# magicat777/Audio-Analyzer-OMEGA

Hardware: AMD Instinct MI355X
Metric: audio frames/sec (multi-res FFT + LUFS + TruePeak) at 1/2/4/8 MI355X (higher is better)
Workload: dtype f32; 1 GPU; cfg2: 256 stereo frames x 16384 samples per GPU; MRFFT 16k/8k/4k/1k + combine(512) + K-weighted LUFS + 4x true peak + meter aggregates; channel_frames_per_gpu=512, frame_samples=16384, target_bins=512, parallelism=frames sharded over 1 GPU(s)

## Files before the change

### audio-analyzer-omega_amd/csrc/capi.cpp

```cpp
#include <hip/hip_runtime.h>

#include <algorithm>
#include <cmath>
#include <cstdarg>
#include <cstdio>
#include <cstdlib>
#include <cstring>
#include <exception>
#include <map>
#include <new>
#include <string>
#include <vector>

#include "../../include/omega.h"
#include "params.hpp"

namespace omega {
hipError_t launch_spectral(int W, const SpectralParams& p, hipStream_t s);
hipError_t launch_mrfft(const SpectralParams& p, hipStream_t s);
hipError_t launch_mrfft_range(const SpectralParams& p, int r0, int r1, hipStream_t s);
hipError_t launch_mrfft_independent(const SpectralParams& p, hipStream_t s);
hipError_t launch_truepeak(int W, const SpectralParams& p, hipStream_t s);
hipError_t launch_truepeak_rf(int W, const SpectralParams& p, hipStream_t s, int extra_lds = 0);
hipError_t launch_mrfft_rf(int n, const SpectralParams& p, int r, hipStream_t s);
// ... 942 lines not shown
    p.seg_post_target = c->seg_par[b];
    v.push_back(p);
    c->cur = b;
  }
  return v;
}

int meters_enqueue(omega_ctx* c, const float* lufs, const float* tp, int64_t n_frames, double* out,
                   hipStream_t stream, hipEvent_t tp_ready, unsigned* wait_ctr = nullptr, unsigned wait_target = 0) {
  bool first = true;
  for (MeterPrepParams p : meter_chunks(c, lufs, tp, n_frames, out)) {
    if (first && wait_ctr) {
      p.wait_ctr = wait_ctr;
      p.wait_target = wait_target;
    }
    HIPC(c, launch_meter_prep(p, stream));
    if (tp_ready && first) HIPC(c, hipStreamWaitEvent(stream, tp_ready, 0));
    HIPC(c, launch_meter_query(p, stream));
    first = false;
  }
  return 0;
}

int flush_meters(omega_ctx* c) {
  if (!c->pend) return 0;
  HIPC(c, hipSetDevice(c->device));
  BatchPlan bp{};
  bp.q_begin = 0;
  bp.q_n = c->pend_nq;
  bp.seg_start[0] = bp.seg_start[1] = bp.multi_start = c->pend_nq;
  SpectralParams sp{};
  KWeightParams kp{};
  const hipError_t le = launch_batch(sp, kp, bp, c->pend_mq, c->pend_nq, c->stream);
  if (le != hipSuccess) return fail(c, OMEGA_EHIP, "meter segment launch: %s", hipGetErrorString(le));
  c->pend = false;
  c->seg_par[c->pend_par] = c->seg_issued + (unsigned)c->pend_nq;
  c->seg_issued += (unsigned)c->pend_nq;
  return 0;
}

bool batch_eligible(omega_ctx* c, const SpectralParams& sp, const KWeightParams& kp, int W, bool do_res, hipStream_t s,
                    int* mr) {
  *mr = -1;
  if (W != 16384 || (c->cap && s == c->cap)) return false;
  if ((kp.lufs_out || kp.weighted_out) && kp.mode != 0) return false;
  if (!do_res) return true;
  if (!c->res_independent) return false;
  for (int r = 0; r < sp.n_res; ++r) {
    if (!sp.comb_out && !sp.res[r].mag_out) continue;
    const int n = sp.res[r].n;
    if (n == 16384) {
      if (*mr >= 0 || !((sp.rf_sizes >> 14) & 1)) return false;
      *mr = r;
    } else if (n < 512 || n > 8192) {
      return false;
    }
  }
  return true;
}

int enqueue_batch(omega_ctx* c, SpectralParams sp, KWeightParams kp, int W, int64_t n_frames, const float* lufs,
                  const float* tp, double* meters, hipStream_t s, int mr, bool do_tp, bool do_kw, bool fold) {
  (void)W;
  const int64_t n = sp.n_cf;
  BatchPlan bp{};
  int seg[2][3], ns[2] = {0, 0};
  auto add = [&](int sg, int role, bool on) {
    if (on) seg[sg][ns[sg]++] = role;
  };
  add(0, 0, do_kw);
  add(0, 2, mr >= 0);
  add(1, 1, do_tp);
  const int64_t groups = (n + 7) / 8;
  int64_t end = 0;
  for (int sg = 0; sg < 2; ++sg) {
    bp.n_roles[sg] = ns[sg] ? ns[sg] : 1;
    for (int i = 0; i < 3; ++i) bp.roles[sg][i] = i < ns[sg] ? seg[sg][i] : 0;
    end += ns[sg] ? 8 * ns[sg] * groups : 0;
    if (end > 0x7FFFFFFF) return fail(c, OMEGA_EINVAL, "batch of %lld channel-frames too large", (long long)n);
    bp.seg_begin[sg + 1] = (int)end;
  }
  bp.mr_res = mr < 0 ? 0 : mr;
  int64_t nwg = 0;
  for (int r = 0; r < sp.n_res; ++r) {
    if (r == mr || (!sp.comb_out && !sp.res[r].mag_out)) continue;
    const int K = sp.res[r].n / 2;
    const int G = K / 16 < 64 ? 64 : K / 16;
    const int fpw = 512 / G;
    bp.multi.res[bp.multi.n_seg] = r;
    bp.multi.wg_begin[bp.multi.n_seg] = (int)nwg;
    ++bp.multi.n_seg;
    nwg += (n + fpw - 1) / fpw;
  }
  const bool in_grid = meters && do_tp && do_kw && n_frames > 0 && n_frames <= kChunkFrames;
  const int64_t n_mq = in_grid ? std::min<int64_t>((n + kBatchWaves - 1) / kBatchWaves, kMeterWgs) : 0;
  fold = fold && in_grid;
  const int64_t q_n = fold ? (c->pend ? c->pend_nq : 0) : n_mq;
  bp.pat = 1;
  bp.multi_n = (int)nwg;
  bp.seg_start[0] = 0;
  bp.seg_start[1] = bp.seg_begin[1];
  bp.multi_start = bp.seg_begin[2];
  const int64_t body_end = end + nwg;
  bp.q_begin = (int)body_end;
  bp.q_n = (int)q_n;
  if (fold) bp.q_begin = bp.multi_start;
  const int64_t grid = body_end + q_n;
  if (grid > 0x7FFFFFFF) return fail(c, OMEGA_EINVAL, "batch of %lld channel-frames too large", (long long)n);
  MeterPrepParams mq{};
  std::vector<MeterPrepParams> mc;
  if (in_grid) {
    const int a = c->cur;
    const unsigned seg_par_was = c->seg_par[a ^ 1];
    if (fold && c->pend) c->seg_par[c->pend_par] = c->seg_issued + (unsigned)c->pend_nq;
    const int cur_was = c->cur;
    mc = meter_chunks(c, lufs, tp, n_frames, meters);
    MeterPrepParams p = mc[0];
    p.q_done = c->d_kw_done + 3;
    const size_t mir_n = (size_t)kChunkFrames * c->cfg.n_channels;
    if (fold && !c->d_mirror) {
      HIPC(c, hipMalloc(&c->d_mirror, 2 * mir_n * sizeof(unsigned long long)));
      HIPC(c, hipMemset(c->d_mirror, 0, 2 * mir_n * sizeof(unsigned long long)));
    }
    const bool mirror = fold;
    const unsigned gen_was = c->mirror_gen;
    if (mirror) {
      c->mirror_gen = c->mirror_gen == 0xFFFFFFFFu ? 2u : c->mirror_gen + 1;
      kp.lufs_mirror = c->d_mirror + (c->mirror_gen & 1) * mir_n;
      kp.mirror_gen = c->mirror_gen;
      p.lufs_mirror = kp.lufs_mirror;
      p.mirror_gen = c->mirror_gen;
    } else {
      kp.kw_done = c->d_kw_done;
      c->kw_issued += (unsigned)n;
      p.wait_ctr = c->d_kw_done;
      p.wait_target = c->kw_issued;
    }
    if (fold && c->tail_ok == 0) {
      int ok = 0;
      HIPC(c, hipDeviceGetAttribute(&ok, hipDeviceAttributeCanUseStreamWaitValue, c->device));
      c->tail_ok = -1;
      if (ok && hipExtMallocWithFlags(reinterpret_cast<void**>(&c->d_tail), 8, hipMallocSignalMemory) == hipSuccess) {
        HIPC(c, hipMemset(c->d_tail, 0, 8));
        c->tail_issued = 0;
        c->tail_ok = 1;
      }
    }
    const bool tail = fold && c->tail_ok > 0;
    if (tail) bp.tail_ctr = c->d_tail;
    if (!fold) HIPC(c, launch_meter_prep(p, c->fork[0]));
    c->side_meters = true;
    mq = mc[0];
    mq.start_ctr = c->d_kw_done + 3;
    mq.start_target = c->prep_issued + (unsigned)p.C;
    if (!fold) {
      sp.tp_done = c->d_kw_done + 2;
      mq.join_ctr = c->d_kw_done + 2;
      mq.join_target = c->tp_issued + (unsigned)n;
    }
    const hipError_t le = launch_batch(sp, kp, bp, fold ? c->pend_mq : mq, (int)grid, s);
    if (le != hipSuccess) {
      if (!fold) {
        (void)hipMemcpy(c->d_kw_done, &c->kw_issued, sizeof(unsigned), hipMemcpyHostToDevice);
        c->prep_issued += (unsigned)p.C;
      } else {
        c->mirror_gen = gen_was;
        c->seg_par[a ^ 1] = seg_par_was;
        c->cur = cur_was;
// ... 2104 lines not shown
```

### audio-analyzer-omega_amd/csrc/fft.hpp

```cpp
#pragma once
#include <hip/hip_runtime.h>
#include <type_traits>
#include <utility>

namespace omega {

constexpr int NT = 256;

template <int A, int B, class F>
__device__ __forceinline__ void static_for(F&& f) {
  if constexpr (A < B) {
    f(std::integral_constant<int, A>{});
    static_for<A + 1, B>(f);
  }
}

constexpr int ilog2(int v) { return v <= 1 ? 0 : 1 + ilog2(v >> 1); }

template <int R>
constexpr int brev(int m) {
  int r = 0;
  for (int b = 0; b < ilog2(R); ++b) r |= ((m >> b) & 1) << (ilog2(R) - 1 - b);
  return r;
}
// ... 70 lines not shown
  for (int n1 = 0; n1 < 4; ++n1) {
    const float2 a0 = v[n1], a1 = v[n1 + 4], a2 = v[n1 + 8], a3 = v[n1 + 12];
    const float2 s02 = make_float2(a0.x + a2.x, a0.y + a2.y), d02 = make_float2(a0.x - a2.x, a0.y - a2.y);
    const float2 s13 = make_float2(a1.x + a3.x, a1.y + a3.y), d13 = make_float2(a1.x - a3.x, a1.y - a3.y);
    v[n1 + 0] = make_float2(s02.x + s13.x, s02.y + s13.y);
    v[n1 + 8] = make_float2(s02.x - s13.x, s02.y - s13.y);
    v[n1 + 4] = make_float2(d02.x + d13.y, d02.y - d13.x);
    v[n1 + 12] = make_float2(d02.x - d13.y, d02.y + d13.x);
  }
  float2 y[16];
#pragma unroll
  for (int i = 0; i < 16; ++i) y[4 * (i & 3) + (i >> 2)] = v[i];
  {
    const float2 a0 = y[0], a1 = y[4], a2 = y[8], a3 = y[12];
    const float2 s02 = make_float2(a0.x + a2.x, a0.y + a2.y), d02 = make_float2(a0.x - a2.x, a0.y - a2.y);
    const float2 s13 = make_float2(a1.x + a3.x, a1.y + a3.y), d13 = make_float2(a1.x - a3.x, a1.y - a3.y);
    v[0] = make_float2(s02.x + s13.x, s02.y + s13.y);
    v[8] = make_float2(s02.x - s13.x, s02.y - s13.y);
    v[4] = make_float2(d02.x + d13.y, d02.y - d13.x);
    v[12] = make_float2(d02.x - d13.y, d02.y + d13.x);
  }
  {
    const float2 a0 = y[1], a1 = y[5], a2 = y[9], a3 = y[13];
    const float p2x = a2.x + a2.y, p2y = a2.y - a2.x, p3x = a3.x + a3.y, p3y = a3.y - a3.x;
    const float2 s02 = make_float2(fmaf(h, p2x, a0.x), fmaf(h, p2y, a0.y));
    const float2 d02 = make_float2(fmaf(-h, p2x, a0.x), fmaf(-h, p2y, a0.y));
    const float2 e = make_float2(fmaf(h, p3x, a1.x), fmaf(h, p3y, a1.y));
    const float2 f = make_float2(fmaf(-h, p3x, a1.x), fmaf(-h, p3y, a1.y));
    const float ux = fmaf(t8, e.y, e.x), uy = fmaf(-t8, e.x, e.y);
    const float wx = fmaf(t8, f.y, f.x), wy = fmaf(-t8, f.x, f.y);
    v[1] = make_float2(fmaf(c8, ux, s02.x), fmaf(c8, uy, s02.y));
    v[9] = make_float2(fmaf(-c8, ux, s02.x), fmaf(-c8, uy, s02.y));
    v[5] = make_float2(fmaf(c8, wy, d02.x), fmaf(-c8, wx, d02.y));
    v[13] = make_float2(fmaf(-c8, wy, d02.x), fmaf(c8, wx, d02.y));
  }
  {
    const float2 a0 = y[2], a1 = y[6], a2 = y[10], a3 = y[14];
    const float2 s02 = make_float2(a0.x + a2.y, a0.y - a2.x), d02 = make_float2(a0.x - a2.y, a0.y + a2.x);
    const float2 e = make_float2(a1.x + a3.y, a1.y - a3.x), f = make_float2(a1.x - a3.y, a1.y + a3.x);
    const float pex = e.x + e.y, pey = e.y - e.x, pfx = f.x + f.y, pfy = f.y - f.x;
    v[2] = make_float2(fmaf(h, pex, s02.x), fmaf(h, pey, s02.y));
    v[10] = make_float2(fmaf(-h, pex, s02.x), fmaf(-h, pey, s02.y));
    v[6] = make_float2(fmaf(h, pfy, d02.x), fmaf(-h, pfx, d02.y));
    v[14] = make_float2(fmaf(-h, pfy, d02.x), fmaf(h, pfx, d02.y));
  }
  {
    const float2 a0 = y[3], a1 = y[7], a2 = y[11], a3 = y[15];
    const float q2s = a2.x + a2.y, q2d = a2.y - a2.x, q3s = a3.x + a3.y, q3d = a3.y - a3.x;
    const float2 s02 = make_float2(fmaf(h, q2d, a0.x), fmaf(-h, q2s, a0.y));
    const float2 d02 = make_float2(fmaf(-h, q2d, a0.x), fmaf(h, q2s, a0.y));
    const float2 e = make_float2(fmaf(h, q3d, a1.x), fmaf(-h, q3s, a1.y));
    const float2 f = make_float2(fmaf(-h, q3d, a1.x), fmaf(h, q3s, a1.y));
    const float ux = fmaf(t8, e.x, e.y), uy = fmaf(t8, e.y, -e.x);
    const float wx = fmaf(t8, f.x, f.y), wy = fmaf(t8, f.y, -f.x);
    v[3] = make_float2(fmaf(c8, ux, s02.x), fmaf(c8, uy, s02.y));
    v[11] = make_float2(fmaf(-c8, ux, s02.x), fmaf(-c8, uy, s02.y));
    v[7] = make_float2(fmaf(c8, wy, d02.x), fmaf(-c8, wx, d02.y));
    v[15] = make_float2(fmaf(-c8, wy, d02.x), fmaf(c8, wx, d02.y));
  }
}

template <int R>
__device__ __forceinline__ void dft_nat(float2* v) {
  if constexpr (R == 16) {
    dft16_fma(v);
  } else {
    dft_dif<R>(v);
    float2 o[R];
    static_for<0, R>([&](auto m) { o[m] = v[brev<R>(m)]; });
    static_for<0, R>([&](auto m) { v[m] = o[m]; });
  }
}

template <int NS, int R>
__device__ __forceinline__ int swz(int i) {
  if constexpr (NS >= 16 || NS == 0) {
    return i;
  } else {
    constexpr int a = ilog2(NS * R), c = ilog2(NS), m = 16 / NS - 1;
    return i ^ (((i >> a) & m) << c);
  }
}

template <int NP>
struct TwReg {
  float2 w[NP > 0 ? NP : 1];
  __device__ __forceinline__ void launder() {
    static_for<0, (NP > 0 ? NP : 1)>([&](auto i) { asm volatile("" : "+v"(w[i].x), "+v"(w[i].y)); });
  }
};

template <int K, int R, int NS, int NTH, bool SYNC_MID, class Load, class Store>
__device__ __forceinline__ void fft_pass(float2 w1, int tid, Load&& load, Store&& store) {
  constexpr int NB = K / R;
  constexpr int B = (NB + NTH - 1) / NTH;
  static_assert(NS == 1 || B == 1, "twiddled passes: one butterfly per thread");
  float2 v[B][R];
  static_for<0, B>([&](auto b) {
    const int j = tid + b * NTH;
    if (NB % NTH == 0 || j < NB) static_for<0, R>([&](auto r) { v[b][r] = load(j + r * NB); });
  });
  if constexpr (SYNC_MID) __syncthreads();
  static_for<0, B>([&](auto b) {
    const int j = tid + b * NTH;
    if (NB % NTH == 0 || j < NB) {
      const int k = j & (NS - 1);
      if constexpr (NS > 1) {
        float2 w = w1;
        static_for<1, R>([&](auto r) {
          v[b][r] = cmul(v[b][r], w);
          if constexpr (r + 1 < R) w = cmul(w, w1);
        });
      }
      dft_nat<R>(v[b]);
      const int base = (j / NS) * NS * R + k;
      static_for<0, R>([&](auto m) { store(base + m * NS, v[b][m]); });
    }
  });
}

template <int K, int NTH, int I, int NS, int PNS, int PR, int... Rs>
struct StockhamChain;
template <int K, int NTH, int I, int NS, int PNS, int PR>
struct StockhamChain<K, NTH, I, NS, PNS, PR> {
  template <class TW>
  static __device__ __forceinline__ void load_tw(const float2*, int, TW&) {}
  template <bool FIRST, bool LAST, bool PP, class TW, class F, class G>
  static __device__ __forceinline__ void run(float2*, float2*, const TW&, int, F&&, G&&) {}
  static __device__ __forceinline__ int out(int i) { return swz<PNS, PR>(i); }
};
template <int K, int NTH, int I, int NS, int PNS, int PR, int R, int... Rs>
struct StockhamChain<K, NTH, I, NS, PNS, PR, R, Rs...> {
  using Next = StockhamChain<K, NTH, I + 1, NS * R, NS, R, Rs...>;
  static constexpr bool kLastPass = sizeof...(Rs) == 0;
  template <class TW>
  static __device__ __forceinline__ void load_tw(const float2* __restrict__ tw, int t, TW& w) {
    w.w[I] = make_float2(1.f, 0.f);
    if constexpr (NS > 1) {
      if ((K / R) % NTH == 0 || t < K / R) w.w[I] = tw[(t & (NS - 1)) * (K / (NS * R))];
    }
    Next::load_tw(tw, t, w);
  }
  template <bool FIRST, bool LAST, bool PP, class TW, class F, class G>
  static __device__ __forceinline__ void run(float2* buf, float2* alt, const TW& w, int t, F&& first, G&& last) {
    float2* dst = PP ? alt : buf;
    auto lds_load = [&](int i) { return buf[swz<PNS, PR>(i)]; };
    auto lds_store = [&](int i, float2 v) { dst[swz<NS, R>(i)] = v; };
    constexpr bool in_global = FIRST && NS == 1;
    constexpr bool out_regs = LAST && kLastPass;
    constexpr bool sync_mid = !in_global && !out_regs && !PP;
    if constexpr (in_global && out_regs)
      fft_pass<K, R, NS, NTH, false>(w.w[I], t, first, last);
    else if constexpr (in_global)
      fft_pass<K, R, NS, NTH, false>(w.w[I], t, first, lds_store);
    else if constexpr (out_regs)
      fft_pass<K, R, NS, NTH, false>(w.w[I], t, lds_load, last);
    else
      fft_pass<K, R, NS, NTH, sync_mid>(w.w[I], t, lds_load, lds_store);
    if constexpr (!out_regs) __syncthreads();
    Next::template run<FIRST, LAST, PP>(dst, PP ? buf : alt, w, t, first, last);
  }
  static __device__ __forceinline__ int out(int i) { return Next::out(i); }
};

template <int K, int NTH, int... Rs>
struct FFTPlan {
  using Chain = StockhamChain<K, NTH, 0, 1, 0, 1, Rs...>;
  using Tw = TwReg<sizeof...(Rs)>;
  static constexpr int kPasses = sizeof...(Rs);
  static __device__ __forceinline__ Tw load_tw(const float2* __restrict__ tw, int t) {
    Tw w;
    Chain::load_tw(tw, t, w);
    return w;
  }
  static __device__ __forceinline__ void run(float2* b, const Tw& w, int t) {
    auto none = [](int) { return make_float2(0.f, 0.f); };
    auto sink = [](int, float2) {};
    Chain::template run<false, false, false>(b, b, w, t, none, sink);
  }
  template <class F>
  static __device__ __forceinline__ void run_from(float2* b, const Tw& w, int t, F&& first) {
    auto sink = [](int, float2) {};
    Chain::template run<true, false, false>(b, b, w, t, first, sink);
  }
  template <class G>
  static __device__ __forceinline__ void run_to(float2* b, const Tw& w, int t, G&& last) {
    auto none = [](int) { return make_float2(0.f, 0.f); };
    Chain::template run<false, true, false>(b, b, w, t, none, last);
  }
  template <class F>
  static __device__ __forceinline__ float2* run_from_pp(float2* b, float2* alt, const Tw& w, int t, F&& first) {
    auto sink = [](int, float2) {};
    Chain::template run<true, false, true>(b, alt, w, t, first, sink);
    return kPasses % 2 ? alt : b;
  }
  template <class G>
  static __device__ __forceinline__ void run_to_pp(float2* b, float2* alt, const Tw& w, int t, G&& last) {
    auto none = [](int) { return make_float2(0.f, 0.f); };
    Chain::template run<false, true, true>(b, alt, w, t, none, last);
  }
  static __device__ __forceinline__ int out(int i) { return Chain::out(i); }
};

template <int K>
constexpr int threads_for() { return K / 16 < 64 ? 64 : (K / 16 > 512 ? 512 : K / 16); }

template <int K, int NTH>
struct BlockFFTPlan;
template <int NTH> struct BlockFFTPlan<8192, NTH> { using type = FFTPlan<8192, NTH, 2, 16, 16, 16>; };
template <> struct BlockFFTPlan<8192, 1024> { using type = FFTPlan<8192, 1024, 2, 8, 8, 8, 8>; };
template <int NTH> struct BlockFFTPlan<4096, NTH> { using type = FFTPlan<4096, NTH, 16, 16, 16>; };
template <int NTH> struct BlockFFTPlan<2048, NTH> { using type = FFTPlan<2048, NTH, 8, 16, 16>; };
template <int NTH> struct BlockFFTPlan<1024, NTH> { using type = FFTPlan<1024, NTH, 4, 16, 16>; };
template <int NTH> struct BlockFFTPlan<512, NTH> { using type = FFTPlan<512, NTH, 2, 16, 16>; };
template <int NTH> struct BlockFFTPlan<256, NTH> { using type = FFTPlan<256, NTH, 16, 16>; };

template <int K, int NTH = threads_for<K>()>
using BlockFFT = typename BlockFFTPlan<K, NTH>::type;

template <int AND, int OR, int XOR>
__device__ __forceinline__ float swizzle32(float v) {
  static_assert(AND < 32 && OR < 32 && XOR < 32, "5-bit masks");
  return __int_as_float(__builtin_amdgcn_ds_swizzle(__float_as_int(v), AND | (OR << 5) | (XOR << 10)));
}
template <bool SHR>
__device__ __forceinline__ float wave_shift1(float v) {
  return __int_as_float(__builtin_amdgcn_update_dpp(0, __float_as_int(v), SHR ? 0x138 : 0x130, 0xF, 0xF, true));
}
__device__ __forceinline__ float read_lane(float v, int l) {
  return __int_as_float(__builtin_amdgcn_readlane(__float_as_int(v), l));
}
__device__ __forceinline__ float wave_sum_sw(float v) {
  v += swizzle32<31, 0, 1>(v);
  v += swizzle32<31, 0, 2>(v);
  v += swizzle32<31, 0, 4>(v);
  v += swizzle32<31, 0, 8>(v);
  v += swizzle32<31, 0, 16>(v);
  return read_lane(v, 0) + read_lane(v, 32);
}

__device__ __forceinline__ float wave_max(float v) {
#pragma unroll
  for (int o = 32; o >= 1; o >>= 1) v = fmaxf(v, __shfl_xor(v, o, 64));
  return v;
}
__device__ __forceinline__ float wave_sum(float v) {
#pragma unroll
  for (int o = 32; o >= 1; o >>= 1) v += __shfl_xor(v, o, 64);
  return v;
}
__device__ __forceinline__ double wave_sum(double v) {
#pragma unroll
// ... 55 lines not shown
```

### audio-analyzer-omega_amd/csrc/params.hpp

```cpp
#pragma once
#include <hip/hip_runtime.h>
#include <stdint.h>

namespace omega {

constexpr int kMaxRes = 4;
constexpr int kMaxLog2 = 15;

struct alignas(16) CombEnt {
  int tm, j;
  float c0, c1;
};

struct ResParam {
  int n;
  int offset;
  const float* win;
  const float* wgt;
  float* mag_out;
  int ent_begin, ent_end;
  float cw;
  int low_band;
  int pair_lo, pair_hi;
};
// ... 75 lines not shown
  const unsigned long long* lufs_mirror;
  unsigned mirror_gen;
  const float* tp;
  int64_t n_frames;
  int C;
  const float* hist_l_in;
  const float* hist_t_in;
  const int* n_l_in;
  const int* n_t_in;
  const unsigned long long* skeys_in;
  const int* n_s_in;
  const uint32_t* t0_in;
  float* hist_l_out;
  float* hist_t_out;
  int* n_l_out;
  int* n_t_out;
  unsigned long long* skeys_out;
  int* n_s_out;
  uint32_t* t0_out;
  int HL, HT;
  int mom_len, short_len, int_len, peak_len;
  float gate;
  float* core;
  MeterExt* ext;
  int* n_core;
  int* n_ext;
  int* gcount;
  double* gsum;
  double* out;
  int parts;
  unsigned* wait_ctr;
  unsigned wait_target;
  unsigned* q_done;
  unsigned* join_ctr;
  unsigned join_target;
  unsigned* start_ctr;
  unsigned start_target;
  unsigned* seg_ctr;
  unsigned seg_pre_target, seg_post_target;
  int poll_limit;
  unsigned* err_word;
};

struct BandParams {
  const float* spec;
  int64_t n, spec_stride;
  int n_bins;
  int n_out;
  const int* starts;
  const int* ends;
  const float* scale;
  const float* bin_scale;
  int op;
  int n_valid;
  float* out;
};

struct ChromaParams {
  const float* spec;
  int64_t n;
  int n_bins;
  double df;
  const float* mat;
  double* out;
};

struct CombineParams {
  const float* mag[kMaxRes];
  int nbins[kMaxRes];
  float cw[kMaxRes];
  int64_t n_cf;
  int T;
  const int* own_off;
  const int* own_rj;
  const float* own_frac;
  float* out;
};

struct MultiPlan {
  int n_seg;
  int res[4];
  int wg_begin[4];
};

struct BatchPlan {
  int seg_begin[3];
  int n_roles[2];
  int roles[2][3];
  int mr_res;
  MultiPlan multi;
  int q_begin, q_n;
  unsigned* tail_ctr;
  int pat;
  int seg_start[2];
  int multi_start, multi_n;
};

struct SpectraParams {
  const float* x;
  int64_t n, stride;
  const float* win;
  const float4* wgen;
  float* mag_out;
  int n_out, n_valid;
  const int* starts;
  const int* ends;
  const float* scale;
  float* bands_out;
  int c_lo, c_hi;
  const float4* cw4;
  const float* cw1;
  const unsigned short* cperm;
  const int* cgoff;
  const float* crec;
  double* chroma_out;
  const float2* tw[kMaxLog2];
};

constexpr int kDrumBands = 7;
constexpr int kDrumHist = 21;
constexpr int kDrumCols = 14;

constexpr int kPostMaxBins = 2048;
constexpr int kEmaSpareRows = 32;
constexpr int kPostMaxBands = 1024;
struct EmaCoef {
  double f, g;
  float f32, g32;
};
struct PostParams {
  const float* in;
  int64_t n, stride;
  int T;
  const double* curve;
  const unsigned char* bass;
  const float* comp[2];
  const float* vsup;
  int be, vs, ve, hs;
  const unsigned* leaf_tab;
  int p_lo, p_hi;
  float p_g;
  const int* bs;
  const int* bend;
  const EmaCoef* sf;
  int nb;
  int flags;
  float bass_boost;
  float* spec_out;
  double* band_out;
  float* band_raw;
  int* frame64;
  double* ema_pre;
  double* ema_end;
  int* content_out;
  double* prev;
  int* has_prev;
  double* prev_out;
  int* has_prev_out;
};

struct DrumParams {
  const float* mag;
  int64_t n, stride;
  int n_bins;
  int bs[kDrumBands], be[kDrumBands];
  int cs, ce;
// ... 172 lines not shown
```

### audio-analyzer-omega_amd/csrc/regfft.hpp

```cpp
#pragma once
#include "fft.hpp"

namespace omega {

__device__ constexpr float kCos128[16] = {
    1.000000000e+00f, 9.987954562e-01f, 9.951847267e-01f, 9.891765100e-01f, 9.807852804e-01f,
    9.700312532e-01f, 9.569403357e-01f, 9.415440652e-01f, 9.238795325e-01f, 9.039892931e-01f,
    8.819212643e-01f, 8.577286100e-01f, 8.314696123e-01f, 8.032075315e-01f, 7.730104534e-01f,
    7.409511254e-01f};
__device__ constexpr float kSin128[16] = {
    0.000000000e+00f, 4.906767433e-02f, 9.801714033e-02f, 1.467304745e-01f, 1.950903220e-01f,
    2.429801799e-01f, 2.902846773e-01f, 3.368898534e-01f, 3.826834324e-01f, 4.275550934e-01f,
    4.713967368e-01f, 5.141027442e-01f, 5.555702330e-01f, 5.956993045e-01f, 6.343932842e-01f,
    6.715589548e-01f};

__device__ __forceinline__ void wave_lds_sync() {
  asm volatile("s_waitcnt lgkmcnt(0)" ::: "memory");
  __builtin_amdgcn_wave_barrier();
}

__device__ __forceinline__ float lane_xor1(float v) {
  return __int_as_float(__builtin_amdgcn_mov_dpp(__float_as_int(v), 0xB1, 0xF, 0xF, true));
}

__device__ __forceinline__ void lane_pair_fmac(float2 (&v)[16], float s) {
  asm volatile(
      "s_nop 1\n"
      "v_fmac_f32_dpp %0, %0, %32 quad_perm:[1,0,3,2] row_mask:0xf bank_mask:0xf\n"
      "v_fmac_f32_dpp %1, %1, %32 quad_perm:[1,0,3,2] row_mask:0xf bank_mask:0xf\n"
      "v_fmac_f32_dpp %2, %2, %32 quad_perm:[1,0,3,2] row_mask:0xf bank_mask:0xf\n"
      "v_fmac_f32_dpp %3, %3, %32 quad_perm:[1,0,3,2] row_mask:0xf bank_mask:0xf\n"
      "v_fmac_f32_dpp %4, %4, %32 quad_perm:[1,0,3,2] row_mask:0xf bank_mask:0xf\n"
      "v_fmac_f32_dpp %5, %5, %32 quad_perm:[1,0,3,2] row_mask:0xf bank_mask:0xf\n"
      "v_fmac_f32_dpp %6, %6, %32 quad_perm:[1,0,3,2] row_mask:0xf bank_mask:0xf\n"
      "v_fmac_f32_dpp %7, %7, %32 quad_perm:[1,0,3,2] row_mask:0xf bank_mask:0xf\n"
      "v_fmac_f32_dpp %8, %8, %32 quad_perm:[1,0,3,2] row_mask:0xf bank_mask:0xf\n"
      "v_fmac_f32_dpp %9, %9, %32 quad_perm:[1,0,3,2] row_mask:0xf bank_mask:0xf\n"
      "v_fmac_f32_dpp %10, %10, %32 quad_perm:[1,0,3,2] row_mask:0xf bank_mask:0xf\n"
      "v_fmac_f32_dpp %11, %11, %32 quad_perm:[1,0,3,2] row_mask:0xf bank_mask:0xf\n"
      "v_fmac_f32_dpp %12, %12, %32 quad_perm:[1,0,3,2] row_mask:0xf bank_mask:0xf\n"
      "v_fmac_f32_dpp %13, %13, %32 quad_perm:[1,0,3,2] row_mask:0xf bank_mask:0xf\n"
      "v_fmac_f32_dpp %14, %14, %32 quad_perm:[1,0,3,2] row_mask:0xf bank_mask:0xf\n"
      "v_fmac_f32_dpp %15, %15, %32 quad_perm:[1,0,3,2] row_mask:0xf bank_mask:0xf\n"
      "v_fmac_f32_dpp %16, %16, %32 quad_perm:[1,0,3,2] row_mask:0xf bank_mask:0xf\n"
      "v_fmac_f32_dpp %17, %17, %32 quad_perm:[1,0,3,2] row_mask:0xf bank_mask:0xf\n"
      "v_fmac_f32_dpp %18, %18, %32 quad_perm:[1,0,3,2] row_mask:0xf bank_mask:0xf\n"
      "v_fmac_f32_dpp %19, %19, %32 quad_perm:[1,0,3,2] row_mask:0xf bank_mask:0xf\n"
      "v_fmac_f32_dpp %20, %20, %32 quad_perm:[1,0,3,2] row_mask:0xf bank_mask:0xf\n"
      "v_fmac_f32_dpp %21, %21, %32 quad_perm:[1,0,3,2] row_mask:0xf bank_mask:0xf\n"
      "v_fmac_f32_dpp %22, %22, %32 quad_perm:[1,0,3,2] row_mask:0xf bank_mask:0xf\n"
      "v_fmac_f32_dpp %23, %23, %32 quad_perm:[1,0,3,2] row_mask:0xf bank_mask:0xf\n"
      "v_fmac_f32_dpp %24, %24, %32 quad_perm:[1,0,3,2] row_mask:0xf bank_mask:0xf\n"
      "v_fmac_f32_dpp %25, %25, %32 quad_perm:[1,0,3,2] row_mask:0xf bank_mask:0xf\n"
      "v_fmac_f32_dpp %26, %26, %32 quad_perm:[1,0,3,2] row_mask:0xf bank_mask:0xf\n"
      "v_fmac_f32_dpp %27, %27, %32 quad_perm:[1,0,3,2] row_mask:0xf bank_mask:0xf\n"
      "v_fmac_f32_dpp %28, %28, %32 quad_perm:[1,0,3,2] row_mask:0xf bank_mask:0xf\n"
      "v_fmac_f32_dpp %29, %29, %32 quad_perm:[1,0,3,2] row_mask:0xf bank_mask:0xf\n"
      "v_fmac_f32_dpp %30, %30, %32 quad_perm:[1,0,3,2] row_mask:0xf bank_mask:0xf\n"
      "v_fmac_f32_dpp %31, %31, %32 quad_perm:[1,0,3,2] row_mask:0xf bank_mask:0xf\n"
      : "+v"(v[0].x), "+v"(v[0].y),
        "+v"(v[1].x), "+v"(v[1].y),
        "+v"(v[2].x), "+v"(v[2].y),
        "+v"(v[3].x), "+v"(v[3].y),
        "+v"(v[4].x), "+v"(v[4].y),
        "+v"(v[5].x), "+v"(v[5].y),
        "+v"(v[6].x), "+v"(v[6].y),
        "+v"(v[7].x), "+v"(v[7].y),
        "+v"(v[8].x), "+v"(v[8].y),
        "+v"(v[9].x), "+v"(v[9].y),
        "+v"(v[10].x), "+v"(v[10].y),
        "+v"(v[11].x), "+v"(v[11].y),
        "+v"(v[12].x), "+v"(v[12].y),
        "+v"(v[13].x), "+v"(v[13].y),
        "+v"(v[14].x), "+v"(v[14].y),
        "+v"(v[15].x), "+v"(v[15].y)
      : "v"(s));
}

struct WinGen {
  float c0, c1, c2;
  float4 base;
  float4 step[8];
  __device__ __forceinline__ WinGen(const float4* __restrict__ g, int t) {
    const float4 c = g[0];
    c0 = c.x;
    c1 = c.y;
    c2 = c.z;
#pragma unroll
    for (int i = 0; i < 8; ++i) step[i] = g[1 + i];
    base = g[9 + t];
  }
  template <int Q, bool C2 = true>
  __device__ __forceinline__ float2 at() const {
    const float4 s4 = step[Q / 2];
    const float cs = (Q & 1) ? s4.z : s4.x, sn = (Q & 1) ? s4.w : s4.y;
    const float C0 = fmaf(base.x, cs, -base.y * sn), C1 = fmaf(base.z, cs, -base.w * sn);
    if constexpr (C2) return make_float2(fmaf(C0, fmaf(c2, C0, c1), c0), fmaf(C1, fmaf(c2, C1, c1), c0));
    else return make_float2(fmaf(C0, c1, c0), fmaf(C1, c1, c0));
  }
};

template <int K>
// ... 203 lines not shown
```

### audio-analyzer-omega_amd/csrc/rfkern.hip

```cpp
#include <cstdlib>

#include "stamps.hpp"

namespace omega {
OMEGA_STAMPS_DECL
OMEGA_WGTRACE_DECL
OMEGA_MARKS_DECL
}

#include "kw.hpp"
#include "meter_query.hpp"
#include "regfft.hpp"
#include "spectral.hpp"

namespace omega {

template <int K>
constexpr size_t t2_offset() { return (RegFFT<K>::kSlots + 8) * sizeof(float2) + 64; }
template <int K>
constexpr size_t lds_bytes() { return t2_offset<K>() + RegFFT<K>::kT2 * sizeof(float2); }
template <int K>
__device__ __forceinline__ float2* t2_table(char* smem) { return reinterpret_cast<float2*>(smem + t2_offset<K>()); }

template <int NTH>
// ... 648 lines not shown
  kw_count_in(kp, tid);
}

__device__ __forceinline__ void batch_meter_role(const MeterPrepParams& mp, int q, int nq, int tid) {
  const int64_t n_out = mp.n_frames * mp.C, step = (int64_t)nq * (kBatchThreads / 64);
  const int64_t o0 = (int64_t)q * (kBatchThreads / 64) + (tid >> 6);
  const int lane = tid & 63;
  OMEGA_MARK(q, 0);
  if (tid == 0) poll_count(mp.start_ctr, mp.start_target, mp.poll_limit, mp.err_word + 1);
  __syncthreads();
  OMEGA_MARK(q, 1);
  for (int64_t o = o0; o < n_out; o += step) meter_query_wave(mp, o / mp.C, (int)(o % mp.C), lane, true, false);
  const float th0 = o0 < n_out ? tp_hist_part(mp, o0 / mp.C, (int)(o0 % mp.C), lane) : -INFINITY;
  OMEGA_MARK(q, 2);
  if (tid == 0) poll_count(mp.join_ctr, mp.join_target, mp.poll_limit, mp.err_word + 1);
  __syncthreads();
  OMEGA_MARK(q, 3);
  const int64_t n_roll = (int64_t)mp.C * mp.HT, roll_step = (int64_t)nq * kBatchThreads;
  int64_t e = (int64_t)q * kBatchThreads + tid;
  float rv = 0.f;
  const int64_t rdst = e < n_roll ? tp_roll_load(mp, e, rv) : -1;
  for (int64_t o = o0; o < n_out; o += step) {
    const int64_t f = o / mp.C;
    const int c = (int)(o % mp.C);
    tp_finish(mp, f, c, lane, o == o0 ? th0 : tp_hist_part(mp, f, c, lane));
  }
  if (rdst >= 0) mp.hist_t_out[rdst] = rv;
  for (e += roll_step; e < n_roll; e += roll_step) {
    const int64_t d = tp_roll_load(mp, e, rv);
    if (d >= 0) mp.hist_t_out[d] = rv;
  }
  if (mp.seg_ctr) {
    asm volatile("s_waitcnt vmcnt(0)" ::: "memory");
    __syncthreads();
    if (tid == 0) __hip_atomic_fetch_add(mp.seg_ctr, 1u, __ATOMIC_RELAXED, __HIP_MEMORY_SCOPE_AGENT);
  }
  OMEGA_MARK(q, 4);
}

__device__ __forceinline__ void batch_body(const SpectralParams& sp, const KWeightParams& kp, const BatchPlan& bp,
                                           const MeterPrepParams& mq, char* smem) {
  const int tid = threadIdx.x;
  const int b = blockIdx.x;
  OMEGA_WG_BEGIN();
  if (bp.tail_ctr && b == (int)gridDim.x - 1 && tid == 0)
    __hip_atomic_fetch_add(bp.tail_ctr, 1u, __ATOMIC_RELAXED, __HIP_MEMORY_SCOPE_SYSTEM);
  if (b >= bp.q_begin && b < bp.q_begin + bp.q_n) {
    batch_meter_role(mq, b - bp.q_begin, bp.q_n, tid);
    OMEGA_WG_END(4);
    return;
  }

  const int len0 = bp.seg_begin[1], len1 = bp.seg_begin[2] - bp.seg_begin[1];
  const int sg = (b >= bp.seg_start[0] && b < bp.seg_start[0] + len0) ? 0
                 : (b >= bp.seg_start[1] && b < bp.seg_start[1] + len1) ? 1 : -1;
  if (sg >= 0) {
    const int j = b - bp.seg_start[sg], nr = bp.n_roles[sg];
    int role;
    int64_t cf;
    if (nr == 2 && bp.pat == 1) {
      const int g = j >> 3, per = g & 7, rb = (0x5A >> per) & 1;
      role = bp.roles[sg][rb];
      const int idx = 4 * (g >> 3) + __popc((rb ? 0x5A : 0xA5) & ((1 << per) - 1));
      cf = (int64_t)idx * 8 + (j & 7);
    } else {
      role = bp.roles[sg][(j >> 3) % nr];
      cf = (int64_t)(j / (8 * nr)) * 8 + (j & 7);
    }
    if (cf >= sp.n_cf) return;
    if (role == 0) {
      batch_kw_role(kp, cf, tid, smem);
    } else if (role == 1) {
      truepeak_rf_body<8192>(sp, cf, tid, smem);
    } else {
      mrfft_rf_body<8192>(sp, bp.mr_res, cf, tid, smem);
    }
    OMEGA_WG_END(role);
    return;
  }
  const MultiPlan& mp = bp.multi;
  const int w = b - bp.multi_start -
                (b >= bp.q_begin + bp.q_n && bp.q_begin < bp.multi_start + bp.multi_n ? bp.q_n : 0);
  if (w < 0 || w >= bp.multi_n) return;
  int s = 0;
  while (s + 1 < mp.n_seg && w >= mp.wg_begin[s + 1]) ++s;
  const int r = mp.res[s];
  const int64_t wg = w - mp.wg_begin[s];
  float2* buf = reinterpret_cast<float2*>(smem);
  switch (sp.res[r].n) {
    case 512: batch_multi<256>(sp, r, wg, tid, buf); break;
    case 1024: batch_multi<512>(sp, r, wg, tid, buf); break;
    case 2048: batch_multi<1024>(sp, r, wg, tid, buf); break;
    case 4096: batch_multi<2048>(sp, r, wg, tid, buf); break;
    case 8192: batch_multi<4096>(sp, r, wg, tid, buf); break;
    default: break;
  }
  OMEGA_WG_END(3 + sp.res[r].n);
}

__global__ __launch_bounds__(kBatchThreads, 4) void batch_kernel(SpectralParams sp, KWeightParams kp, BatchPlan bp,
                                                                 MeterPrepParams mq) {
  extern __shared__ __attribute__((aligned(16))) char smem[];
  batch_body(sp, kp, bp, mq, smem);
}

hipError_t launch_batch(const SpectralParams& sp, const KWeightParams& kp, const BatchPlan& bp, const MeterPrepParams& mq,
                        int grid, hipStream_t s) {
  hipLaunchKernelGGL(batch_kernel, dim3((unsigned)grid), dim3(kBatchThreads), lds_bytes<8192>(), s, sp, kp, bp, mq);
  return hipGetLastError();
}

}
```

### audio-analyzer-omega_amd/csrc/spectral.hip

```cpp
#include "stamps.hpp"

namespace omega {
OMEGA_STAMPS_DECL
}

#include "spectral.hpp"

namespace omega {

template <int K, int NTH = threads_for<K>()>
__global__ __launch_bounds__(NTH, 2 * NTH / 256) void mrfft_kernel(SpectralParams p, int r) {
  extern __shared__ __attribute__((aligned(16))) char smem[];
  mrfft_frame<K, NTH>(p, r, blockIdx.x, true, threadIdx.x, reinterpret_cast<float2*>(smem));
}

constexpr int kMultiThreads = 256;

template <int K>
__device__ __forceinline__ void mrfft_multi_seg(const SpectralParams& p, int r, int64_t wg, float2* smem) {
  constexpr int G = threads_for<K>();
  constexpr int FPW = kMultiThreads / G;
  const int grp = threadIdx.x / G;
  const int64_t cf = wg * FPW + grp;
  const bool valid = cf < p.n_cf;
  mrfft_frame<K, G>(p, r, valid ? cf : p.n_cf - 1, valid, threadIdx.x % G, smem + grp * K);
}

__global__ __launch_bounds__(kMultiThreads) void mrfft_multi_kernel(SpectralParams p, MultiPlan mp) {
  extern __shared__ __attribute__((aligned(16))) char smem[];
  float2* buf = reinterpret_cast<float2*>(smem);
  int s = 0;
  while (s + 1 < mp.n_seg && (int)blockIdx.x >= mp.wg_begin[s + 1]) ++s;
  const int r = mp.res[s];
  const int64_t wg = (int64_t)blockIdx.x - mp.wg_begin[s];
  switch (p.res[r].n) {
    case 512: mrfft_multi_seg<256>(p, r, wg, buf); break;
    case 1024: mrfft_multi_seg<512>(p, r, wg, buf); break;
    case 2048: mrfft_multi_seg<1024>(p, r, wg, buf); break;
    case 4096: mrfft_multi_seg<2048>(p, r, wg, buf); break;
    case 8192: mrfft_multi_seg<4096>(p, r, wg, buf); break;
    default: break;
  }
}

template <int K, int NTH = tp_threads<K>()>
__global__ __launch_bounds__(NTH, (NTH / 256 > 2 ? NTH / 256 : 2)) void truepeak_kernel(SpectralParams p) {
  extern __shared__ __attribute__((aligned(16))) char smem[];
  float2* bufA = reinterpret_cast<float2*>(smem);
  truepeak_body<K, NTH>(p, blockIdx.x, threadIdx.x, bufA, bufA + K, reinterpret_cast<float*>(smem + 2 * K * sizeof(float2)));
}

template <int K, int NTH = threads_for<K>()>
__global__ __launch_bounds__(NTH, 2 * NTH / 256) void rfft_kernel(RfftParams p) {
  using FFT = BlockFFT<K, NTH>;
  extern __shared__ __attribute__((aligned(16))) char smem[];
  float2* buf = reinterpret_cast<float2*>(smem);
  const int tid = threadIdx.x;
  const int64_t i = blockIdx.x;
  const float2* x2 = reinterpret_cast<const float2*>(p.x + i * (2 * K));
  const float2* w2 = reinterpret_cast<const float2*>(p.win);
  FFT::run_from(buf, FFT::load_tw(p.tw[ilog2(K)], tid), tid, [&](int n) {
    const float2 a = x2[n], w = w2[n];
    return make_float2(a.x * w.x, a.y * w.y);
  });
  const float2* __restrict__ twN = p.tw[ilog2(2 * K)];
  float2* cp = p.cplx ? reinterpret_cast<float2*>(p.cplx) + i * (K + 1) : nullptr;
  float* mp = p.mag ? p.mag + i * (K + 1) : nullptr;
  for (int k = tid; k < K / 2; k += NTH) {
    float2 xk, xkk;
    if (k == 0) {
      const float2 z = buf[FFT::out(0)];
      xk = make_float2(z.x + z.y, 0.f);
      xkk = make_float2(z.x - z.y, 0.f);
      const float2 xm = cconj(buf[FFT::out(K / 2)]);
      if (cp) cp[K / 2] = xm;
      if (mp) mp[K / 2] = cabs(xm);
    } else {
      untangle(buf[FFT::out(k)], buf[FFT::out(K - k)], twN[k], xk, xkk);
    }
    if (cp) {
      cp[k] = xk;
      cp[K - k] = xkk;
    }
    if (mp) {
      mp[k] = cabs(xk);
      mp[K - k] = cabs(xkk);
    }
  }
}

__global__ __launch_bounds__(256) void combine_kernel(CombineParams p) {
  const int64_t cf = blockIdx.y;
  for (int t = blockIdx.x * 256 + threadIdx.x; t < p.T; t += gridDim.x * 256) {
    float acc = 0.f, ws = 0.f;
    for (int q = p.own_off[t]; q < p.own_off[t + 1]; ++q) {
      const int rj = p.own_rj[q];
      const int r = rj >> 24, j = rj & 0xFFFFFF;
      const float* m = p.mag[r];
      if (!m) continue;
      m += cf * p.nbins[r];
      const float fr = p.own_frac[q];
      const float v = fr != 0.f ? fmaf(fr, m[j + 1] - m[j], m[j]) : m[j];
      acc = fmaf(v, p.cw[r], acc);
      ws += p.cw[r];
    }
    p.out[cf * p.T + t] = ws > 0.f ? acc / ws : 0.f;
  }
}

constexpr int kSmallThreads = 64;
__global__ __launch_bounds__(kSmallThreads) void mrfft_small_kernel(SpectralParams p, int r) {
  __shared__ float xs[256];
  __shared__ float mag[129];
  const ResParam& rp = p.res[r];
  const int N = rp.n, K = N / 2, t = threadIdx.x;
// ... 137 lines not shown
```

### audio-analyzer-omega_amd/csrc/spectral.hpp

```cpp
#pragma once
#include "fft.hpp"
#include "params.hpp"
#include "stamps.hpp"

namespace omega {

__device__ __forceinline__ float cabs(float2 z) { return __builtin_amdgcn_sqrtf(fmaf(z.x, z.x, z.y * z.y)); }

__device__ __forceinline__ void untangle(float2 a, float2 b, float2 w, float2& xk, float2& xkk) {
  const float2 E = make_float2(0.5f * (a.x + b.x), 0.5f * (a.y - b.y));
  const float2 O = make_float2(0.5f * (a.y + b.y), -0.5f * (a.x - b.x));
  const float2 wo = cmul(w, O);
  xk = cadd(E, wo);
  xkk = cconj(csub(E, wo));
}

template <int K, int NTH>
__device__ __forceinline__ int magidx(int k) {
  return k == K ? 2 * BlockFFT<K, NTH>::out(0) : 2 * BlockFFT<K, NTH>::out(k) + 1;
}

template <int K, int NTH>
__device__ __forceinline__ void rfft_magnitudes(float2* buf, const float2* __restrict__ twN, int tid, int k0 = 0,
                                                int k1 = K / 2) {
  using FFT = BlockFFT<K, NTH>;
  float* mag = reinterpret_cast<float*>(buf);
  for (int k = k0 + tid; k < k1; k += NTH) {
    if (k == 0) {
      const float2 z = buf[FFT::out(0)];
      const float2 zm = buf[FFT::out(K / 2)];
      mag[magidx<K, NTH>(0)] = fabsf(z.x + z.y);
      mag[magidx<K, NTH>(K)] = fabsf(z.x - z.y);
      mag[magidx<K, NTH>(K / 2)] = cabs(zm);
    } else {
      float2 xk, xkk;
      untangle(buf[FFT::out(k)], buf[FFT::out(K - k)], twN[k], xk, xkk);
      mag[magidx<K, NTH>(k)] = cabs(xk);
      mag[magidx<K, NTH>(K - k)] = cabs(xkk);
    }
  }
  __syncthreads();
}

template <int K, int NTH>
__device__ __forceinline__ void mrfft_frame(const SpectralParams& p, int r, int64_t cf, bool valid, int tid, float2* buf) {
  const int64_t f = cf / p.C, c = cf % p.C;
  const ResParam& rp = p.res[r];
  const float* __restrict__ x = p.x + f * p.frame_stride + c * p.chan_stride + rp.offset;
  const float2* x2 = reinterpret_cast<const float2*>(x);
  const float2* w2 = reinterpret_cast<const float2*>(rp.win);
  using FFT = BlockFFT<K, NTH>;
  OMEGA_STAMP(10 + 4 * (ilog2(K) - 9));
  const typename FFT::Tw tw = FFT::load_tw(p.tw[ilog2(K)], tid);
  constexpr int EP = NTH >= 256 ? 1 : (NTH >= 128 ? 256 / NTH : 512 / NTH);
  CombEnt ent[EP];
  static_for<0, EP>([&](auto i) {
    const int e = rp.ent_begin + tid + i * NTH;
    if (p.comb_out && e < rp.ent_end) ent[i] = p.ent[e];
  });
  FFT::run_from(buf, tw, tid, [&](int i) {
    const float2 a = valid ? x2[i] : make_float2(0.f, 0.f), w = w2[i];
    return make_float2(a.x * w.x, a.y * w.y);
  });
  OMEGA_STAMP(11 + 4 * (ilog2(K) - 9));
  const bool pair_range = !rp.mag_out && rp.pair_hi > 0;
  if (!rp.mag_out && !pair_range) {
    if (!valid || !p.comb_out) return;
    const float2* __restrict__ twN = p.tw[ilog2(2 * K)];
    auto mag_at = [&](int j) -> float {
      const float2 a = buf[FFT::out(j == K ? 0 : j)];
      if (j == 0) return fabsf(a.x + a.y);
      if (j == K) return fabsf(a.x - a.y);
      if (j == K / 2) return cabs(a);
      float2 xk, xkk;
      untangle(a, buf[FFT::out(K - j)], twN[j], xk, xkk);
      return cabs(xk);
    };
    float* o = p.comb_out + cf * p.T;
    auto apply = [&](const CombEnt& en) {
      const int t = en.tm & 0xFFFFFF, op = en.tm >> 24;
      if (op == 2) {
        o[t] = 0.f;
        return;
      }
      const float v = fmaf(en.c1, mag_at(en.j + 1), en.c0 * mag_at(en.j));
      if (op == 0)
        o[t] = v;
      else
        o[t] += v;
    };
    static_for<0, EP>([&](auto i) {
      if (rp.ent_begin + tid + i * NTH < rp.ent_end) apply(ent[i]);
    });
    for (int e = rp.ent_begin + tid + EP * NTH; e < rp.ent_end; e += NTH) apply(p.ent[e]);
    return;
  }
  rfft_magnitudes<K, NTH>(buf, p.tw[ilog2(2 * K)], tid, pair_range ? rp.pair_lo : 0, pair_range ? rp.pair_hi : K / 2);
  OMEGA_STAMP(12 + 4 * (ilog2(K) - 9));
  if (!valid) return;
  const float* mag = reinterpret_cast<const float*>(buf);
  const float* __restrict__ wgt = rp.wgt;
  if (rp.mag_out) {
    float* o = rp.mag_out + cf * (K + 1);
    for (int k = tid; k <= K; k += NTH) o[k] = mag[magidx<K, NTH>(k)] * wgt[k];
  }
  if (p.comb_out) {
    float* o = p.comb_out + cf * p.T;
    auto apply = [&](const CombEnt& en) {
      const int t = en.tm & 0xFFFFFF, op = en.tm >> 24;
      const float v = fmaf(en.c1, mag[magidx<K, NTH>(en.j + 1)], en.c0 * mag[magidx<K, NTH>(en.j)]);
      if (op == 0)
        o[t] = v;
      else if (op == 1)
        o[t] += v;
      else
        o[t] = 0.f;
    };
    static_for<0, EP>([&](auto i) {
      if (rp.ent_begin + tid + i * NTH < rp.ent_end) apply(ent[i]);
    });
    for (int e = rp.ent_begin + tid + EP * NTH; e < rp.ent_end; e += NTH) apply(p.ent[e]);
  }
  OMEGA_STAMP(13 + 4 * (ilog2(K) - 9));
}

template <int K>
constexpr int tp_threads() { return K == 8192 ? 1024 : threads_for<K>(); }

template <int K, int NTH>
__device__ __forceinline__ void truepeak_body(const SpectralParams& p, int64_t cf, int tid, float2* bufA, float2* bufB,
                                              float* red) {
  constexpr int M = 2 * K;
  using FFT = BlockFFT<K, NTH>;
  const int64_t f = cf / p.C, c = cf % p.C;
  const float2* x2 = reinterpret_cast<const float2*>(p.x + f * p.frame_stride + c * p.chan_stride);
  float mx = 0.f;
  OMEGA_STAMP(0);
  const typename FFT::Tw tw = FFT::load_tw(p.tw[ilog2(K)], tid);
  const float2* buf = FFT::run_from_pp(bufA, bufB, tw, tid, [&](int i) {
    const float2 a = x2[i];
    mx = fmaxf(mx, fmaxf(fabsf(a.x), fabsf(a.y)));
    return a;
  });
  OMEGA_STAMP(1);
  const float2* __restrict__ twM = p.tw[ilog2(M)];
  constexpr int NP = K / 2;
  constexpr int PB = (NP + NTH - 1) / NTH;
  float2 Xlo[PB], Xhi[PB];
  float2 Xmid = make_float2(0.f, 0.f);
  static_for<0, PB>([&](auto b) {
    const int k = tid + b * NTH;
    if (NP % NTH == 0 || k < NP) {
      const int kk = k == 0 ? K / 2 : K - k;
      const float2 a = buf[FFT::out(k)], bz = buf[FFT::out(kk)];
      float2 lo, hi;
      untangle(a, bz, twM[k], lo, hi);
      if (k == 0) Xmid = cconj(bz);
      Xlo[b] = k == 0 ? make_float2(a.x + a.y, 0.f) : lo;
      Xhi[b] = k == 0 ? make_float2(a.x - a.y, 0.f) : hi;
    }
  });
  const float2* __restrict__ rot = p.rot;
  constexpr float kS2 = 7.071067812e-01f;
  float2 rk[PB], ek[PB];
  static_for<0, PB>([&](auto b) {
    const int k = tid + b * NTH;
    rk[b] = (NP % NTH == 0 || k < NP) ? rot[k] : make_float2(1.f, 0.f);
    const float2 r2 = cmul(rk[b], rk[b]);
    ek[b] = cmul(r2, r2);
  });
  const float2 rh = rot[K / 2];
  float fmx = 0.f;
  constexpr bool kOddPasses = FFT::kPasses % 2 == 1;
  OMEGA_STAMP(2);
  int zsel = buf == bufA ? 1 : 0;
#pragma unroll 1
  for (int P = 1; P <= 3; ++P) {
// ... 61 lines not shown
```

Before: 8.433 million channel-frames/s.

## Prefetch FFT inputs and combine twiddles, use wave-level syncs, reorder small segments

Front-loads the global loads of input samples, window and combine-stage twiddles into registers before the first FFT pass, so the first pass reads from registers and twiddle latency overlaps the FFT. Replaces __syncthreads with a wave-local LDS wait when the FFT runs on a single wavefront. Reorders the small-resolution workgroup segments by an estimated per-workgroup cost so the heavier ones are dispatched first. Replaces the segment search loop with branchless arithmetic. Prefetching raises register pressure and may reduce occupancy.

Result: no change. 8.475 million channel-frames/s, median of 6 (+0.5%).

```diff
diff --git a/audio-analyzer-omega_amd/csrc/capi.cpp b/audio-analyzer-omega_amd/csrc/capi.cpp
--- a/audio-analyzer-omega_amd/csrc/capi.cpp
+++ b/audio-analyzer-omega_amd/csrc/capi.cpp
@@ -1048,8 +1048,15 @@
   }
   bp.mr_res = mr < 0 ? 0 : mr;
   int64_t nwg = 0;
+  int small[kMaxRes], sizes[kMaxRes], n_small = 0;
   for (int r = 0; r < sp.n_res; ++r) {
     if (r == mr || (!sp.comb_out && !sp.res[r].mag_out)) continue;
+    small[n_small] = r;
+    sizes[n_small++] = sp.res[r].n;
+  }
+  order_small_segments(small, sizes, n_small);
+  for (int i = 0; i < n_small; ++i) {
+    const int r = small[i];
     const int K = sp.res[r].n / 2;
     const int G = K / 16 < 64 ? 64 : K / 16;
     const int fpw = 512 / G;
diff --git a/audio-analyzer-omega_amd/csrc/fft.hpp b/audio-analyzer-omega_amd/csrc/fft.hpp
--- a/audio-analyzer-omega_amd/csrc/fft.hpp
+++ b/audio-analyzer-omega_amd/csrc/fft.hpp
@@ -176,6 +176,17 @@
   }
 }
 
+__device__ __forceinline__ void wave_lds_sync() {
+  asm volatile("s_waitcnt lgkmcnt(0)" ::: "memory");
+  __builtin_amdgcn_wave_barrier();
+}
+
+template <int NTH>
+__device__ __forceinline__ void group_sync() {
+  if constexpr (NTH <= 64) wave_lds_sync();
+  else __syncthreads();
+}
+
 template <int NP>
 struct TwReg {
   float2 w[NP > 0 ? NP : 1];
@@ -183,6 +194,14 @@
     static_for<0, (NP > 0 ? NP : 1)>([&](auto i) { asm volatile("" : "+v"(w[i].x), "+v"(w[i].y)); });
   }
 };
+
+template <int Q, class Load>
+__device__ __forceinline__ float2 pass_load(Load&& load, int i) {
+  if constexpr (std::is_invocable_v<Load, int, std::integral_constant<int, Q>>)
+    return load(i, std::integral_constant<int, Q>{});
+  else
+    return load(i);
+}
 
 template <int K, int R, int NS, int NTH, bool SYNC_MID, class Load, class Store>
 __device__ __forceinline__ void fft_pass(float2 w1, int tid, Load&& load, Store&& store) {
@@ -192,9 +211,10 @@
   float2 v[B][R];
   static_for<0, B>([&](auto b) {
     const int j = tid + b * NTH;
-    if (NB % NTH == 0 || j < NB) static_for<0, R>([&](auto r) { v[b][r] = load(j + r * NB); });
+    if (NB % NTH == 0 || j < NB)
+      static_for<0, R>([&](auto r) { v[b][r] = pass_load<NB % NTH == 0 ? b + r * B : 0>(load, j + r * NB); });
   });
-  if constexpr (SYNC_MID) __syncthreads();
+  if constexpr (SYNC_MID) group_sync<NTH>();
   static_for<0, B>([&](auto b) {
     const int j = tid + b * NTH;
     if (NB % NTH == 0 || j < NB) {
@@ -251,10 +271,15 @@
       fft_pass<K, R, NS, NTH, false>(w.w[I], t, lds_load, last);
     else
       fft_pass<K, R, NS, NTH, sync_mid>(w.w[I], t, lds_load, lds_store);
-    if constexpr (!out_regs) __syncthreads();
+    if constexpr (!out_regs) group_sync<NTH>();
     Next::template run<FIRST, LAST, PP>(dst, PP ? buf : alt, w, t, first, last);
   }
   static __device__ __forceinline__ int out(int i) { return Next::out(i); }
+};
+
+template <int R0, int...>
+struct first_of {
+  static constexpr int value = R0;
 };
 
 template <int K, int NTH, int... Rs>
@@ -262,6 +287,8 @@
   using Chain = StockhamChain<K, NTH, 0, 1, 0, 1, Rs...>;
   using Tw = TwReg<sizeof...(Rs)>;
   static constexpr int kPasses = sizeof...(Rs);
+  static constexpr int kFirstRadix = first_of<Rs...>::value;
+  static constexpr bool kEvenFirst = (K / kFirstRadix) % NTH == 0;
   static __device__ __forceinline__ Tw load_tw(const float2* __restrict__ tw, int t) {
     Tw w;
     Chain::load_tw(tw, t, w);
diff --git a/audio-analyzer-omega_amd/csrc/params.hpp b/audio-analyzer-omega_amd/csrc/params.hpp
--- a/audio-analyzer-omega_amd/csrc/params.hpp
+++ b/audio-analyzer-omega_amd/csrc/params.hpp
@@ -181,6 +181,24 @@
   int res[4];
   int wg_begin[4];
 };
+__host__ __device__ inline int multi_segment(const MultiPlan& mp, int w) {
+  return (int)(1 < mp.n_seg && w >= mp.wg_begin[1]) + (int)(2 < mp.n_seg && w >= mp.wg_begin[2]) +
+         (int)(3 < mp.n_seg && w >= mp.wg_begin[3]);
+}
+
+inline float small_wg_cost(int n) { return n >= 8192 ? 10.7f : (n >= 4096 ? 8.1f : 7.8f); }
+inline void order_small_segments(int* res, int* n, int count) {
+  for (int i = 1; i < count; ++i) {
+    const int r = res[i], m = n[i];
+    int j = i;
+    for (; j > 0 && small_wg_cost(n[j - 1]) < small_wg_cost(m); --j) {
+      res[j] = res[j - 1];
+      n[j] = n[j - 1];
+    }
+    res[j] = r;
+    n[j] = m;
+  }
+}
 
 struct BatchPlan {
   int seg_begin[3];
diff --git a/audio-analyzer-omega_amd/csrc/regfft.hpp b/audio-analyzer-omega_amd/csrc/regfft.hpp
--- a/audio-analyzer-omega_amd/csrc/regfft.hpp
+++ b/audio-analyzer-omega_amd/csrc/regfft.hpp
@@ -13,11 +13,6 @@
     2.429801799e-01f, 2.902846773e-01f, 3.368898534e-01f, 3.826834324e-01f, 4.275550934e-01f,
     4.713967368e-01f, 5.141027442e-01f, 5.555702330e-01f, 5.956993045e-01f, 6.343932842e-01f,
     6.715589548e-01f};
-
-__device__ __forceinline__ void wave_lds_sync() {
-  asm volatile("s_waitcnt lgkmcnt(0)" ::: "memory");
-  __builtin_amdgcn_wave_barrier();
-}
 
 __device__ __forceinline__ float lane_xor1(float v) {
   return __int_as_float(__builtin_amdgcn_mov_dpp(__float_as_int(v), 0xB1, 0xF, 0xF, true));
diff --git a/audio-analyzer-omega_amd/csrc/rfkern.hip b/audio-analyzer-omega_amd/csrc/rfkern.hip
--- a/audio-analyzer-omega_amd/csrc/rfkern.hip
+++ b/audio-analyzer-omega_amd/csrc/rfkern.hip
@@ -754,8 +754,7 @@
   const int w = b - bp.multi_start -
                 (b >= bp.q_begin + bp.q_n && bp.q_begin < bp.multi_start + bp.multi_n ? bp.q_n : 0);
   if (w < 0 || w >= bp.multi_n) return;
-  int s = 0;
-  while (s + 1 < mp.n_seg && w >= mp.wg_begin[s + 1]) ++s;
+  const int s = multi_segment(mp, w);
   const int r = mp.res[s];
   const int64_t wg = w - mp.wg_begin[s];
   float2* buf = reinterpret_cast<float2*>(smem);
diff --git a/audio-analyzer-omega_amd/csrc/spectral.hip b/audio-analyzer-omega_amd/csrc/spectral.hip
--- a/audio-analyzer-omega_amd/csrc/spectral.hip
+++ b/audio-analyzer-omega_amd/csrc/spectral.hip
@@ -29,8 +29,7 @@
 __global__ __launch_bounds__(kMultiThreads) void mrfft_multi_kernel(SpectralParams p, MultiPlan mp) {
   extern __shared__ __attribute__((aligned(16))) char smem[];
   float2* buf = reinterpret_cast<float2*>(smem);
-  int s = 0;
-  while (s + 1 < mp.n_seg && (int)blockIdx.x >= mp.wg_begin[s + 1]) ++s;
+  const int s = multi_segment(mp, (int)blockIdx.x);
   const int r = mp.res[s];
   const int64_t wg = (int64_t)blockIdx.x - mp.wg_begin[s];
   switch (p.res[r].n) {
diff --git a/audio-analyzer-omega_amd/csrc/spectral.hpp b/audio-analyzer-omega_amd/csrc/spectral.hpp
--- a/audio-analyzer-omega_amd/csrc/spectral.hpp
+++ b/audio-analyzer-omega_amd/csrc/spectral.hpp
@@ -39,7 +39,7 @@
       mag[magidx<K, NTH>(K - k)] = cabs(xkk);
     }
   }
-  __syncthreads();
+  group_sync<NTH>();
 }
 
 template <int K, int NTH>
@@ -51,48 +51,80 @@
   const float2* w2 = reinterpret_cast<const float2*>(rp.win);
   using FFT = BlockFFT<K, NTH>;
   OMEGA_STAMP(10 + 4 * (ilog2(K) - 9));
-  const typename FFT::Tw tw = FFT::load_tw(p.tw[ilog2(K)], tid);
   constexpr int EP = NTH >= 256 ? 1 : (NTH >= 128 ? 256 / NTH : 512 / NTH);
   CombEnt ent[EP];
   static_for<0, EP>([&](auto i) {
     const int e = rp.ent_begin + tid + i * NTH;
+    if constexpr (i < (EP < 2 ? EP : 2)) ent[i] = CombEnt{};
     if (p.comb_out && e < rp.ent_end) ent[i] = p.ent[e];
   });
-  FFT::run_from(buf, tw, tid, [&](int i) {
-    const float2 a = valid ? x2[i] : make_float2(0.f, 0.f), w = w2[i];
-    return make_float2(a.x * w.x, a.y * w.y);
-  });
+  asm volatile("" ::: "memory");
+  const typename FFT::Tw tw = FFT::load_tw(p.tw[ilog2(K)], tid);
+  const bool pair_range = !rp.mag_out && rp.pair_hi > 0;
+  const bool comb_only = !rp.mag_out && !pair_range;
+  const float2* __restrict__ twN = p.tw[ilog2(2 * K)];
+  constexpr int PF = EP < 2 ? EP : 2;
+  float2 tj[PF][2];
+  auto fetch_tj = [&]() {
+    static_for<0, PF>([&](auto i) {
+      tj[i][0] = twN[ent[i].j & (2 * K - 1)];
+      tj[i][1] = twN[(ent[i].j + 1) & (2 * K - 1)];
+    });
+  };
+  if constexpr (FFT::kEvenFirst) {
+    constexpr int NX = K / NTH;
+    float2 xa[NX], wa[NX];
+    static_for<0, NX>([&](auto q) {
+      const int i = tid + q * NTH;
+      xa[q] = valid ? x2[i] : make_float2(0.f, 0.f);
+      wa[q] = w2[i];
+    });
+    asm volatile("" ::: "memory");
+    if (comb_only) fetch_tj();
+    asm volatile("" ::: "memory");
+    FFT::run_from(buf, tw, tid, [&](int, auto q) { return make_float2(xa[q].x * wa[q].x, xa[q].y * wa[q].y); });
+  } else {
+    if (comb_only) fetch_tj();
+    FFT::run_from(buf, tw, tid, [&](int i) {
+      const float2 a = valid ? x2[i] : make_float2(0.f, 0.f), w = w2[i];
+      return make_float2(a.x * w.x, a.y * w.y);
+    });
+  }
   OMEGA_STAMP(11 + 4 * (ilog2(K) - 9));
-  const bool pair_range = !rp.mag_out && rp.pair_hi > 0;
-  if (!rp.mag_out && !pair_range) {
+  if (comb_only) {
     if (!valid || !p.comb_out) return;
-    const float2* __restrict__ twN = p.tw[ilog2(2 * K)];
-    auto mag_at = [&](int j) -> float {
+    auto mag_at = [&](int j, float2 wj) -> float {
       const float2 a = buf[FFT::out(j == K ? 0 : j)];
       if (j == 0) return fabsf(a.x + a.y);
       if (j == K) return fabsf(a.x - a.y);
       if (j == K / 2) return cabs(a);
       float2 xk, xkk;
-      untangle(a, buf[FFT::out(K - j)], twN[j], xk, xkk);
+      untangle(a, buf[FFT::out(K - j)], wj, xk, xkk);
       return cabs(xk);
     };
     float* o = p.comb_out + cf * p.T;
-    auto apply = [&](const CombEnt& en) {
+    auto apply = [&](const CombEnt& en, float2 w0, float2 w1) {
       const int t = en.tm & 0xFFFFFF, op = en.tm >> 24;
       if (op == 2) {
         o[t] = 0.f;
         return;
       }
-      const float v = fmaf(en.c1, mag_at(en.j + 1), en.c0 * mag_at(en.j));
+      const float v = fmaf(en.c1, mag_at(en.j + 1, w1), en.c0 * mag_at(en.j, w0));
       if (op == 0)
         o[t] = v;
       else
         o[t] += v;
     };
+    auto apply_ld = [&](const CombEnt& en) {
+      apply(en, twN[en.j & (2 * K - 1)], twN[(en.j + 1) & (2 * K - 1)]);
+    };
     static_for<0, EP>([&](auto i) {
-      if (rp.ent_begin + tid + i * NTH < rp.ent_end) apply(ent[i]);
-    });
-    for (int e = rp.ent_begin + tid + EP * NTH; e < rp.ent_end; e += NTH) apply(p.ent[e]);
+      if (rp.ent_begin + tid + i * NTH < rp.ent_end) {
+        if constexpr (i < PF) apply(ent[i], tj[i][0], tj[i][1]);
+        else apply_ld(ent[i]);
+      }
+    });
+    for (int e = rp.ent_begin + tid + EP * NTH; e < rp.ent_end; e += NTH) apply_ld(p.ent[e]);
     return;
   }
   rfft_magnitudes<K, NTH>(buf, p.tw[ilog2(2 * K)], tid, pair_range ? rp.pair_lo : 0, pair_range ? rp.pair_hi : K / 2);
```
